# omerbt/Splice

Hardware: AMD Instinct MI355X
Metric: opt_steps_per_sec (higher is better)
Workload: dtype bf16

## Files before the change

### include/splice_hip.h

```cpp
#ifndef SPLICE_HIP_H
#define SPLICE_HIP_H
#include <stddef.h>
#include <stdint.h>

#ifdef __cplusplus
extern "C" {
#endif

typedef uint16_t splice_bf16;
typedef void* splice_stream_t;

#define SPLICE_OK 0
#define SPLICE_ERR_ARG -1
#define SPLICE_ERR_HIP -2
#define SPLICE_ERR_STATE -3
#define SPLICE_ERR_NOMEM -4

int splice_version(void);
int splice_dev_switches(void);
const char* splice_last_error(void);

typedef struct splice_gemm_epilogue {
    const float* bias;
    const float* resid;
// ... 281 lines not shown
                       float* out_f32, size_t os, splice_bf16* out_bf, splice_bf16* pre_bf, const splice_bf16* aux, size_t ps, int pre_lo,
                       splice_stream_t stream);

typedef struct splice_gen_conv_args {
    const float* in;
    const float* w;
    const float* bias;
    float* out;
    size_t in_nstride, in_cstride, out_nstride, out_cstride, w_jstride, w_cstride, p_nstride;
    int N, Cin, Hi, Wi, Cout, Ho, Wo, ks, stride, pad;
    int reflect, act, transposed, accumulate;
    float* ws;
    size_t ws_floats;
    int p_group, defer_reduce;
} splice_gen_conv_args;
#define SPLICE_GEN_CONV_FORM_INTS 5
int splice_gen_conv(const splice_gen_conv_args* args, int* form_out, splice_stream_t stream);
int splice_gen_conv_pair(const splice_gen_conv_args* a, const splice_gen_conv_args* b, int* forms_out, splice_stream_t stream);
int splice_gen_conv_reflect_dgrad(const splice_gen_conv_args* args, float* pad_scratch, size_t scratch_floats, splice_stream_t stream);

typedef struct splice_gen_wgrad_args {
    const float* x;
    const float* dy;
    float* ws;
    size_t ws_floats;
    size_t x_nstride, x_cstride, dy_nstride, dy_cstride;
    int N, Cin, Hi, Wi, Cout, Ho, Wo, ks, stride, pad, reflect;
} splice_gen_wgrad_args;
#define SPLICE_GEN_WGRAD_FORM_INTS 6
size_t splice_gen_conv_wgrad_ws_floats(int N, int Cin, int Cout, int ks, int Ho, int Wo);
int splice_gen_conv_wgrad(const splice_gen_wgrad_args* args, float* dw, int accumulate, int n_img, size_t p_nstride, int* form_out,
                          splice_stream_t stream);
int splice_gen_wgrad_reduce(const float* partials, int n, int chunks, float* dw, int accumulate, int n_img, size_t p_nstride, splice_stream_t stream);

typedef struct splice_gen_bn_args {
    float* y;
    float* out;
    size_t y_nstride, out_nstride;
    int N, C, HW, batch;
    const float* gamma;
    const float* beta;
    float eps, slope;
    size_t p_nstride;
    float* part;
    size_t part_floats;
    float* mean;
    float* rstd;
    const float* up_src;
    float* up_d_src;
    size_t up_src_ns, up_d_src_ns;
    int up_c0, up_h, up_w, up_Ho, up_Wo;
    const float* slabs;
    const float* bias;
    int ksplit;
    const float* da;
    float* dy;
    size_t da_nstride, dy_nstride;
    float* dgamma;
    float* dbeta;
    int accumulate;
    const float* da_slabs;
    int da_ksplit, da_accumulate;
    float* pre_y;
    size_t pre_y_ns;
    const float* pre_slabs;
    const float* pre_bias;
// ... 30 lines not shown
```

### splice_amd/_lib.py

```python
import ctypes as C
import os

_HERE = os.path.dirname(os.path.abspath(__file__))
LIB_PATH = os.path.join(_HERE, "libsplice_hip.so")

_lib = None


class GemmEpilogue(C.Structure):
    _fields_ = [
        ("bias", C.c_void_p), ("resid", C.c_void_p), ("ldr", C.c_int), ("resid_mod", C.c_int),
        ("out_f32", C.c_void_p), ("ldo", C.c_int),
        ("out_bf", C.c_void_p), ("ldbf", C.c_int),
        ("out_bf_t", C.c_void_p), ("ldt", C.c_int),
        ("out_pre", C.c_void_p), ("ldp", C.c_int), ("pre_row_lo", C.c_int),
        ("aux", C.c_void_p), ("ldaux", C.c_int),
        ("out_f32_cols", C.c_void_p), ("ld_cols", C.c_int), ("col_lo", C.c_int), ("col_hi", C.c_int),
        ("alpha", C.c_float), ("ksplit", C.c_int), ("slab_stride", C.c_longlong),
        ("rd_other", C.c_void_p), ("ld_rd", C.c_int), ("rd_rows", C.c_int), ("rowdot", C.c_void_p),
        ("row_scale", C.c_void_p), ("col_scale", C.c_void_p),
        ("out_f8", C.c_void_p), ("ld8", C.c_int),
        ("out_f8_t", C.c_void_p), ("ldt8", C.c_int),
    ]

# ... 79 lines not shown
    "splice_gemm_nt_fp8": ([_u, _vp, _i, _vp, _i, _i, _i, _i, C.POINTER(GemmEpilogue), _vp], _i),
    "splice_quantize_rows_fp8": ([_vp, _i, _vp, _i, _vp, _i, _i, _vp], _i),
    "splice_gemm_splitk_slabs": ([_i, _i], _i),
    "splice_gemm_force_tile": ([_i], _i),
    "splice_attention_variant": ([_i], _i),
    "splice_attention_qfold": ([_i], _i),
    "splice_attention_bwd_variant": ([_i], _i),
    "splice_layernorm_fwd": ([_vp, _vp, _vp, _vp, _vp, _vp, _i, _i, _f, _vp], _i),
    "splice_layernorm_bwd": ([_vp, _vp, _vp, _vp, _vp, _vp, _vp, _vp, _i, _i, _vp], _i),
    "splice_attention_fwd": ([_vp, _vp, _i, _i, _i, _i, _i, _i, _f, _vp, _vp, _vp], _i),
    "splice_attention_fwd_fp8": ([_vp, _vp, _i, _i, _i, _i, _i, _i, _f, _vp, _vp, _vp], _i),
    "splice_attention_bwd": ([_vp, _vp, _i, _i, _i, _i, _i, _i, _f, _vp, _vp, _vp, _vp, _vp, _vp, _vp], _i),
    "splice_attention_probs": ([_vp, _i, _i, _i, _i, _i, _f, _vp, _vp, _vp], _i),
    "splice_augment_structure": ([_vp, _vp, _vp, _i, _i, _i, _i, C.POINTER(C.c_int), C.POINTER(C.c_float), _f, _vp], _i),
    "splice_keys_selfsim_ws_bytes": ([_i, _i], _sz),
    "splice_keys_selfsim_fwd": ([_vp, _i, _i, _i, _f, _vp, _vp, _vp], _i),
    "splice_keys_selfsim_bwd": ([_vp, _vp, _i, _i, _f, _vp, _i, _i, _vp, _vp], _i),
    "splice_mse": ([_vp, _i, _vp, _i, _i, _i, _f, _vp, _vp, _i, _vp], _i),
    "splice_selfsim_loss_pairs_ws_bytes": ([_i, _i, _i], _sz),
    "splice_selfsim_loss_pairs": ([_vp, _vp, _i, _sz, _vp, _i, _sz, _i, _i, _i, _f, _vp, _i, _f, _vp, _sz, _vp, _i, _sz, _vp, _vp], _i),
    "splice_mse_pairs": ([_vp, _i, _sz, _vp, _i, _sz, _i, _i, _f, _f, _vp, _sz, _vp, _i, _sz, _i, _vp, _vp], _i),
    "splice_total_loss_pairs": ([_vp, _sz, _i, _f, _f, _f, _f, _f, _vp, _i, _i, _i, _i, _i, _vp, _i, _i, _vp], _i),
    "splice_attn_cls_fwd": ([_vp, _vp, _i, _i, _i, _i, _i, _i, _f, _vp, _vp, _vp], _i),
    "splice_attn_cls_bwd": ([_vp, _vp, _i, _i, _i, _i, _i, _i, _f, _vp, _vp, _i, _sz, _vp, _vp], _i),
    "splice_ln_rows_fwd": ([_vp, _sz, _vp, _vp, _vp, _sz, _vp, _vp, _sz, _i, _i, _f, _vp, _i, _sz, _vp, _vp, _sz, _vp], _i),
    "splice_ln_rows_bwd": ([_vp, _sz, _vp, _sz, _vp, _vp, _vp, _sz, _vp, _vp, _i, _i, _i, _sz, _vp], _i),
    "splice_rows_finish": ([_i, _vp, _i, _sz, _i, _i, _vp, _vp, _sz, _vp, _sz, _vp, _vp, _vp, _sz, _i, _vp], _i),
    "splice_gen_conv": ([C.POINTER(GenConvArgs), C.POINTER(_i), _vp], _i),
    "splice_gen_conv_pair": ([C.POINTER(GenConvArgs), C.POINTER(GenConvArgs), C.POINTER(_i), _vp], _i),
    "splice_gen_conv_reflect_dgrad": ([C.POINTER(GenConvArgs), _vp, _sz, _vp], _i),
    "splice_gen_conv_wgrad_ws_floats": ([_i, _i, _i, _i, _i, _i], _sz),
    "splice_gen_conv_wgrad": ([C.POINTER(GenWgradArgs), _vp, _i, _i, _sz, C.POINTER(_i), _vp], _i),
    "splice_gen_wgrad_reduce": ([_vp, _i, _i, _vp, _i, _i, _sz, _vp], _i),
    "splice_gen_bn_small_instance": ([_i], _i),
    "splice_gen_bn_form": ([_i, _i, _sz, _i, C.POINTER(_i)], _i),
    "splice_gen_bn_part_floats": ([_i, _i], _sz),
    "splice_gen_bn_fwd": ([C.POINTER(GenBnArgs), _vp], _i),
    "splice_gen_bn_bwd": ([C.POINTER(GenBnArgs), _vp], _i),
    "splice_gen_upsample2x_fwd": ([_vp, _sz, _vp, _sz, _i, _i, _i, _i, _i, _i, _vp], _i),
    "splice_gen_upsample2x_bwd": ([_vp, _sz, _vp, _sz, _i, _i, _i, _i, _i, _i, _vp], _i),
    "splice_gen_sigmoid_bias_part_floats": ([_i, _i], _sz),
    "splice_gen_sigmoid_bwd_bias": ([_vp, _vp, _vp, _i, _i, _i, _vp, _sz, _sz, _i, C.POINTER(_i), _vp], _i),
    "splice_patchify": ([_vp, _vp, _i, _i, _i, _i, _i, _i, _vp], _i),
    "splice_unpatchify": ([_vp, _vp, _i, _i, _i, _i, _i, _i, _vp], _i),
    "splice_cast_f32_bf16": ([_vp, _vp, _sz, _vp], _i),
    "splice_cast_bf16_f32": ([_vp, _vp, _sz, _vp], _i),
    "splice_transpose_f32_bf16": ([_vp, _vp, _i, _i, _i, _vp], _i),
    "splice_resize_bilinear_fwd": ([_vp, _vp, _i, _i, _i, _i, _i, _vp], _i),
    "splice_resize_bilinear_bwd": ([_vp, _vp, _i, _i, _i, _i, _i, _vp], _i),
    "splice_vit_create": ([_i, _i, _i, _i, C.POINTER(_vp)], _i),
    "splice_vit_destroy": ([_vp], None),
    "splice_vit_set_param": ([_vp, C.c_char_p, _vp, C.c_longlong, _vp], _i),
    "splice_vit_params_complete": ([_vp], _i),
    "splice_vit_enable_fp8": ([_vp, _vp], _i),
    "splice_vit_ctx_create": ([_vp, _i, _i, _i, _vp, _i, _vp, C.POINTER(_vp)], _i),
    "splice_vit_ctx_destroy": ([_vp], None),
    "splice_vit_ctx_info": ([_vp, C.POINTER(_i), C.POINTER(_i), C.POINTER(_i)], _i),
    "splice_vit_ctx_set_top_cls_only": ([_vp, _i], _i),
    "splice_vit_ctx_set_fp8": ([_vp, _i], _i),
    "splice_vit_forward": ([_vp, _vp, _i, _vp], _i),
    "splice_vit_forward_ex": ([_vp, _vp, _i, _i, _vp], _i),
    "splice_vit_forward_passes": ([_vp, _vp, _i, _i, _i, _i, _vp], _i),
    "splice_vit_get_tensor": ([_vp, _i, _i, C.POINTER(_vp)], _i),
    "splice_vit_qscale": ([_vp], C.c_float),
    "splice_vit_read_tensor": ([_vp, _i, _i, _vp, _sz, _vp], _i),
    "splice_vit_backward": ([_vp, _i, _i, C.POINTER(_vp), C.POINTER(_vp), C.POINTER(_vp), _vp, _i, _vp], _i),
# ... 102 lines not shown
```

### splice_amd/csrc/capi.hip

```cpp
#include <stdarg.h>
#include <stdio.h>

#include "gen_kernels.h"
#include "kernels.h"

static thread_local char g_err[512] = "";

void splice_set_error(const char* fmt, ...) {
    va_list ap;
    va_start(ap, fmt);
    vsnprintf(g_err, sizeof(g_err), fmt, ap);
    va_end(ap);
}

static int finish(int rc, const char* what) {
    if (rc != SPLICE_OK) {
        splice_set_error("%s: invalid argument", what);
        return rc;
    }
    const hipError_t e = hipGetLastError();
    if (e != hipSuccess) {
        splice_set_error("%s: HIP error %d (%s)", what, (int)e, hipGetErrorString(e));
        return SPLICE_ERR_HIP;
    }
// ... 248 lines not shown
}
size_t splice_gen_conv_wgrad_ws_floats(int N, int Cin, int Cout, int ks, int Ho, int Wo) {
    if (N < 1 || Cin < 1 || Cout < 1 || ks < 1 || Ho < 1 || Wo < 1) return 0;
    int ppc = 0, cpi = 0;
    return (size_t)wgrad_chunks(N, Ho, Wo, &ppc, &cpi) * Cout * Cin * ks * ks;
}
int splice_gen_conv_wgrad(const splice_gen_wgrad_args* args, float* dw, int accumulate, int n_img, size_t p_nstride, int* form_out, splice_stream_t stream) {
    const char* who = "splice_gen_conv_wgrad";
    if (!gen_wgrad_args_ok(args) || !dw || !args->ws) return finish(SPLICE_ERR_ARG, who);
    const size_t n = (size_t)args->Cout * args->Cin * args->ks * args->ks;
    if (n > 0x7fffffffULL || args->ws_floats < splice_gen_conv_wgrad_ws_floats(args->N, args->Cin, args->Cout, args->ks, args->Ho, args->Wo))
        return finish(SPLICE_ERR_ARG, who);
    if (p_nstride ? (n_img != args->N || p_nstride < n) : n_img != 1) return finish(SPLICE_ERR_ARG, who);
    WgradArgs a = {};
    a.x = args->x; a.dy = args->dy; a.ws = args->ws;
    a.x_nstride = args->x_nstride; a.x_cstride = args->x_cstride; a.dy_nstride = args->dy_nstride; a.dy_cstride = args->dy_cstride;
    a.N = args->N; a.Cin = args->Cin; a.Hi = args->Hi; a.Wi = args->Wi; a.Cout = args->Cout; a.Ho = args->Ho; a.Wo = args->Wo;
    a.ks = args->ks; a.stride = args->stride; a.pad = args->pad; a.reflect = args->reflect;
    WgradBatchPair pair = {};
    int chunks = 0;
    int rc = conv_wgrad_add(&pair, a, &chunks);
    if (rc != SPLICE_OK) return finish(rc, who);
    WgradReduceAll r = {};
    r.count = 1; r.n[0] = (int)n; r.chunks[0] = chunks; r.ws_off[0] = 0; r.dw_off[0] = 0;
    if (form_out) {
        const WgradBatch& b = pair.tile.count ? pair.tile : pair.big.count ? pair.big : pair.small;
        form_out[0] = pair.tile.count ? 2 : pair.big.count ? 1 : 0;
        form_out[1] = b.d[0].variant;
        form_out[2] = b.d[0].pix_per_chunk;
        form_out[3] = chunks;
        form_out[4] = !((reinterpret_cast<size_t>(args->ws) | reinterpret_cast<size_t>(dw)) & 15) && p_nstride % 4 == 0 && n % 4 == 0;
        form_out[5] = b.total_wgs;
    }
    rc = conv_wgrad_batched_launch(pair, ST(stream));
    if (rc != SPLICE_OK) return finish(rc, who);
    return finish(wgrad_reduce_all_launch(r, args->ws, dw, accumulate, ST(stream), n_img, p_nstride), who);
}

int splice_gen_wgrad_reduce(const float* partials, int n, int chunks, float* dw, int accumulate, int n_img, size_t p_nstride, splice_stream_t stream) {
    const char* who = "splice_gen_wgrad_reduce";
    if (!partials || !dw || n < 1 || chunks < 0 || n_img < 1 || n_img > 65535 || (long long)n * (chunks > 0 ? chunks : 1) > 0x7fffffffLL) return finish(SPLICE_ERR_ARG, who);
    if (p_nstride ? (chunks % n_img || p_nstride < (size_t)n) : n_img != 1) return finish(SPLICE_ERR_ARG, who);
    WgradReduceAll r = {};
    r.count = 1; r.n[0] = n; r.chunks[0] = chunks; r.ws_off[0] = 0; r.dw_off[0] = 0;
    return finish(wgrad_reduce_all_launch(r, partials, dw, accumulate, ST(stream), n_img, p_nstride), who);
}

int splice_gen_bn_small_instance(int mask) { return finish(bn_small_force_instance(mask), "splice_gen_bn_small_instance"); }
int splice_gen_bn_form(int HW, int N, size_t p_nstride, int batch, int* out) {
    if (HW < 1 || N < 1 || batch < 0 || !out) return finish(SPLICE_ERR_ARG, "splice_gen_bn_form");
    const BnForm f = bn_form(HW, N, p_nstride, batch);
    out[0] = (int)f.kind; out[1] = f.hosts_pre; out[2] = f.fwd_takes_slabs; out[3] = f.bwd_takes_slabs;
    out[4] = f.fwd_fuses_upsample; out[5] = f.bwd_fuses_upsample; out[6] = f.sign_from_y;
    return SPLICE_OK;
}
size_t splice_gen_bn_part_floats(int N, int C) { return N < 1 || C < 1 ? 0 : (size_t)bn_part_floats(N, C); }
static bool gen_bn_fill(const splice_gen_bn_args* g, bool bwd, BnArgs* a, BnUpsample* up, BnPre* pre, BnSlabs* sl) {
    if (!g || !g->y || !g->out || !g->gamma || !g->mean || !g->rstd) return false;
    if (g->N < 1 || g->C < 1 || g->HW < 1 || g->N > 65535 || g->C > 65535 || g->batch < 0 || g->batch > 8) return false;
    if (g->batch && (g->N % g->batch || (g->N != g->batch && !g->p_nstride))) return false;
    if (g->N > 1 && (g->y_nstride < (size_t)g->C * g->HW || g->out_nstride < (size_t)g->C * g->HW)) return false;
    const BnForm f = bn_form(g->HW, g->N, g->p_nstride, g->batch);
    const bool two_stage = f.kind == BnForm::TWO_STAGE || f.kind == BnForm::TWO_STAGE_VEC;
    if (two_stage && (!g->part || g->part_floats < (size_t)bn_part_floats(g->N, g->C))) return false;
    if (!bwd && !g->beta) return false;
    if (bwd && ((f.sign_from_y && !g->beta) || !g->da || !g->dy || !g->dgamma || !g->dbeta)) return false;
    if (bwd && g->N > 1 && (g->da_nstride < (size_t)g->C * g->HW || g->dy_nstride < (size_t)g->C * g->HW)) return false;
    a->y = g->y; a->y_nstride = g->y_nstride; a->out = g->out; a->out_nstride = g->out_nstride;
    a->N = g->N; a->C = g->C; a->HW = g->HW; a->gamma = g->gamma; a->beta = g->beta; a->eps = g->eps; a->slope = g->slope;
    a->p_nstride = g->p_nstride; a->batch = g->batch; a->part = g->part; a->mean = g->mean; a->rstd = g->rstd;
// ... 95 lines not shown
```

### splice_amd/csrc/gen_kernels.h

```cpp
#pragma once
#include "common.h"

struct ConvArgs {
    const float* in;
    const float* w;
    const float* bias;
    float* out;
    size_t in_nstride, in_cstride, out_nstride, out_cstride;
    size_t w_jstride, w_cstride;
    size_t p_nstride;
    int N, Cin, Hi, Wi, Cout, Ho, Wo;
    int ks, stride, pad;
    int reflect;
    int act;
    int transposed;
    int accumulate;
    float* ws;
    size_t ws_floats;
    int ksplit;
    int p_group;
    int defer_reduce;
};
int conv_launch(const ConvArgs& a, hipStream_t s, int* ksplit_out = nullptr);
void conv_form_report(const ConvArgs& a, int* form);
int conv_pair_launch(ConvArgs a, ConvArgs b, hipStream_t s, int* ksplit_a = nullptr, int* ksplit_b = nullptr);
int conv_reflect_dgrad_launch(ConvArgs a, float* pad_scratch, hipStream_t s);

struct WgradArgs {
    const float* x;
    const float* dy;
    float* ws;
    size_t x_nstride, x_cstride, dy_nstride, dy_cstride;
    int N, Cin, Hi, Wi, Cout, Ho, Wo, ks, stride, pad;
    int pix_per_chunk, chunks_per_img;
    int reflect;
};
int wgrad_chunks(int N, int Ho, int Wo, int* pix_per_chunk, int* chunks_per_img);
constexpr int WGRAD_BATCH_MAX = 32;
struct WgradDesc {
    const float* x; const float* dy; float* ws;
    uint32_t x_nstride, x_cstride, dy_nstride, dy_cstride;
    uint16_t Cin, Cout, Hi, Wi, Ho, Wo;
    uint8_t ks, stride, pad, variant;
    uint16_t pix_per_chunk, chunks_per_img;
    uint32_t wg_begin, chunks;
    uint32_t reflect;
};
struct WgradBatch { int count; int total_wgs; WgradDesc d[WGRAD_BATCH_MAX]; };
struct WgradBatchPair { WgradBatch small, big, tile; };
int conv_wgrad_add(WgradBatchPair* b, WgradArgs a, int* chunks_out);
int conv_wgrad_batched_launch(const WgradBatchPair& b, hipStream_t s);

constexpr int WGRAD_MAX_LAYERS = 64;
struct WgradReduceAll {
    long long prefix[WGRAD_MAX_LAYERS + 1];
    long long ws_off[WGRAD_MAX_LAYERS];
    long long dw_off[WGRAD_MAX_LAYERS];
    int n[WGRAD_MAX_LAYERS], chunks[WGRAD_MAX_LAYERS];
    long long total;
    int count;
    unsigned char vec[WGRAD_MAX_LAYERS];
};
int wgrad_reduce_all_launch(const WgradReduceAll& d, const float* ws, float* grads, int accumulate, hipStream_t s, int n_img = 1, size_t p_nstride = 0);

int bn_part_floats(int N, int C);
struct BnUpsample {
    const float* src = nullptr; size_t src_ns = 0;
    float* d_src = nullptr; size_t d_src_ns = 0;
    int c0 = 0, h = 0, w = 0, Ho = 0, Wo = 0;
};
struct BnPre {
    const float* y = nullptr; size_t y_ns = 0;
    const float* slabs = nullptr; int ksplit = 0;
    const float* bias = nullptr;
    const float* gamma = nullptr; const float* beta = nullptr;
    float* mean = nullptr; float* rstd = nullptr;
    float slope = 0.2f;
    int C = 0;
    float* dy = nullptr;
    float* dgamma = nullptr; float* dbeta = nullptr;
};
struct BnSlabs {
    const float* slabs = nullptr;
    int ksplit = 0, accumulate = 0;
// ... 53 lines not shown
```

### splice_amd/csrc/gen_wgrad.hip

```cpp
#include "gen_device.h"
#include <cstdlib>

constexpr int WG_PC = 64;
constexpr int WG_LD = WG_PC + 2;
constexpr int WG_XS_FLOATS = 3 * 16 * WG_LD;
constexpr int WG_DS_FLOATS = 8 * 16 * WG_LD;
template <int KS, int NI, bool ROWS = false>
__device__ __forceinline__ void conv_wgrad_body(const WgradArgs& a, int chunk, int ktile_in, float* Xs, float* Ds) {
    constexpr int T = ROWS ? KS : KS * KS;
    constexpr int CK = (ROWS || KS == 3) ? 4 : 16;
    constexpr int KT = CK * T;
    const int ktile = ROWS ? ktile_in / KS : ktile_in;
    const int krow = ROWS ? ktile_in % KS : 0;
    constexpr int NJ = (KT + 15) / 16;
    constexpr int PC = WG_PC;
    constexpr int LD = WG_LD;
    constexpr int NQ = (NI * NJ + 3) / 4;
    constexpr int NA = KT / 4;
    constexpr int ND = NI * 16 * PC / 256;
    const int tid = threadIdx.x, lane = tid & 63, wave = tid >> 6;
    const int c0 = ktile * CK;
    const int HWo = a.Ho * a.Wo;
    const int chunks_per_img = a.chunks_per_img;
    const int img = chunk / chunks_per_img, ch_in_img = chunk % chunks_per_img;
    const float* x = a.x + (size_t)img * a.x_nstride + (size_t)c0 * a.x_cstride;
    const float* dy = a.dy + (size_t)img * a.dy_nstride;
    f32x4 acc[NQ];
#pragma unroll
    for (int q = 0; q < NQ; ++q) acc[q] = f32x4{0.f, 0.f, 0.f, 0.f};
    for (int e = tid; e < (NJ * 16 - KT) * LD; e += 256) Xs[KT * LD + e] = 0.f;
    const int pl = tid & 63;
    const int p_begin = ch_in_img * a.pix_per_chunk;
    const int p_end = min(p_begin + a.pix_per_chunk, HWo);
    const int wave_g = (KS == 3 && NI == 8) ? __builtin_amdgcn_readfirstlane(wave) : wave;
    int g_coff[NA], g_dy[NA], g_dx[NA];
    unsigned g_cok = 0;
#pragma unroll
    for (int i = 0; i < NA; ++i) {
        const int k = wave_g + 4 * i;
        const int cl = k / T, tap = k % T;
        g_coff[i] = (int)(cl * a.x_cstride);
        g_dy[i] = (ROWS ? krow : tap / KS) - a.pad;
        g_dx[i] = (ROWS ? tap : tap % KS) - a.pad;
        if (c0 + cl < a.Cin) g_cok |= 1u << i;
    }
    float xv[NA], dv[ND];
    const __amdgpu_buffer_rsrc_t rx = __builtin_amdgcn_make_buffer_rsrc(const_cast<float*>(x), 0, 0x7FFFFFFF, 0x00020000);
    const __amdgpu_buffer_rsrc_t rdy = __builtin_amdgcn_make_buffer_rsrc(const_cast<float*>(dy), 0, 0x7FFFFFFF, 0x00020000);
    int d_vo[ND];
#pragma unroll
    for (int t = 0; t < ND; ++t) {
        const int e = tid + 256 * t;
        const int n = e / PC, q = e % PC;
        d_vo[t] = n < a.Cout ? (int)((n * a.dy_cstride + q) * 4) : (int)0x80000000;
    }
    auto fetch = [&](int pb) {
        const int p = pb + pl;
        const bool pvalid = p < p_end;
        const int oy = pvalid ? p / a.Wo : 0, ox = pvalid ? p % a.Wo : 0;
        const int by = oy * a.stride, bx = ox * a.stride;
#pragma unroll
        for (int i = 0; i < NA; ++i) {
            int sy = by + g_dy[i], sx = bx + g_dx[i];
            if (a.reflect) {
                sy = sy < 0 ? -sy : (sy >= a.Hi ? 2 * (a.Hi - 1) - sy : sy);
                sx = sx < 0 ? -sx : (sx >= a.Wi ? 2 * (a.Wi - 1) - sx : sx);
            }
            const bool ok = pvalid && ((g_cok >> i) & 1u) && (unsigned)sy < (unsigned)a.Hi && (unsigned)sx < (unsigned)a.Wi;
            const int vo = ok ? (g_coff[i] + sy * a.Wi + sx) * 4 : (int)0x80000000;
            xv[i] = __builtin_bit_cast(float, __builtin_amdgcn_raw_buffer_load_b32(rx, vo, 0, 0));
        }
        if (pb + PC <= p_end) {
            const int so = __builtin_amdgcn_readfirstlane(pb * 4);
#pragma unroll
            for (int t = 0; t < ND; ++t) dv[t] = __builtin_bit_cast(float, __builtin_amdgcn_raw_buffer_load_b32(rdy, d_vo[t], so, 0));
        } else {
#pragma unroll
            for (int t = 0; t < ND; ++t) {
                const int e = tid + 256 * t;
                const int n = e / PC, q = e % PC;
                const int pp = pb + q;
                dv[t] = (n < a.Cout && pp < p_end) ? dy[(size_t)n * a.dy_cstride + pp] : 0.f;
            }
        }
    };
    fetch(p_begin);
    constexpr int WB = 4, NB = PC / 4 / WB;
    [[maybe_unused]] int lds_rd = (lane & 15) * LD + (lane >> 4);
    for (int pb = p_begin; pb < p_end; pb += PC) {
        if constexpr (NI < 4) asm volatile("" : "+v"(lds_rd));
        __syncthreads();
#pragma unroll
        for (int i = 0; i < NA; ++i) Xs[(wave + 4 * i) * LD + pl] = xv[i];
#pragma unroll
        for (int t = 0; t < ND; ++t) {
            const int e = tid + 256 * t;
            Ds[(e / PC) * LD + (e % PC)] = dv[t];
        }
        __syncthreads();
        if (pb + PC < p_end) fetch(pb + PC);
#pragma unroll
        for (int q = 0; q < NQ; ++q) {
            const int pair = wave + 4 * q;
            if (pair < NI * NJ) {
                const int fi = pair / NJ, fj = pair % NJ;
                if constexpr (NI >= 4) {
#pragma unroll
                    for (int s4 = 0; s4 < PC / 4; ++s4) {
                        const float av = Ds[(fi * 16 + (lane & 15)) * LD + s4 * 4 + (lane >> 4)];
                        const float bv = Xs[(fj * 16 + (lane & 15)) * LD + s4 * 4 + (lane >> 4)];
                        acc[q] = mfma4(av, bv, acc[q]);
                    }
                } else {
                    const int d_rd = lds_rd + fi * 16 * LD, x_rd = lds_rd + fj * 16 * LD;
                    float af[2][WB], bf[2][WB];
#pragma unroll
                    for (int t = 0; t < WB; ++t) { af[0][t] = Ds[d_rd + t * 4]; bf[0][t] = Xs[x_rd + t * 4]; }
#pragma unroll
                    for (int b = 0; b < NB; ++b) {
                        if (b + 1 < NB) {
#pragma unroll
                            for (int t = 0; t < WB; ++t) { af[(b + 1) & 1][t] = Ds[d_rd + ((b + 1) * WB + t) * 4]; bf[(b + 1) & 1][t] = Xs[x_rd + ((b + 1) * WB + t) * 4]; }
                        }
                        __builtin_amdgcn_sched_barrier(0);
#pragma unroll
                        for (int t = 0; t < WB; ++t) acc[q] = mfma4(af[b & 1][t], bf[b & 1][t], acc[q]);
                        __builtin_amdgcn_sched_barrier(0);
                    }
                }
            }
        }
    }
    constexpr int TT = KS * KS;
    float* ws = a.ws + (size_t)chunk * a.Cout * a.Cin * TT;
#pragma unroll
    for (int q = 0; q < NQ; ++q) {
        const int pair = wave + 4 * q;
        if (pair < NI * NJ) {
            const int fi = pair / NJ, fj = pair % NJ;
            const int k = fj * 16 + (lane & 15);
            const int cl = k / T, tap = k % T;
            if (k < KT && c0 + cl < a.Cin) {
#pragma unroll
                for (int r = 0; r < 4; ++r) {
                    const int n = fi * 16 + (lane >> 4) * 4 + r;
                    if (n < a.Cout) ws[((size_t)n * a.Cin + c0 + cl) * TT + (ROWS ? krow * KS + tap : tap)] = acc[q][r];
                }
            }
        }
    }
}

__device__ __forceinline__ void wgrad_loaded(float& x) { asm volatile("" : "+v"(x) : : "memory"); }
template <class Load>
__device__ __forceinline__ float wgrad_chunk_sum(int chunks, Load&& ld) {
    float s0 = 0.f, s1 = 0.f, s2 = 0.f, s3 = 0.f;
    int c = 0;
#pragma unroll 1
    for (; c + 31 < chunks; c += 32) {
        float v[32];
#pragma unroll
        for (int u = 0; u < 32; ++u) v[u] = ld(c + u);
#pragma unroll
        for (int u = 0; u < 32; ++u) wgrad_loaded(v[u]);
#pragma unroll
        for (int u = 0; u < 32; u += 4) { s0 += v[u]; s1 += v[u + 1]; s2 += v[u + 2]; s3 += v[u + 3]; }
    }
    for (; c + 15 < chunks; c += 16) {
        float v[16];
#pragma unroll
// ... 71 lines not shown
            const float4 v0 = *reinterpret_cast<const float4*>(p + (size_t)c * n), v1 = *reinterpret_cast<const float4*>(p + (size_t)(c + 1) * n),
                         v2 = *reinterpret_cast<const float4*>(p + (size_t)(c + 2) * n), v3 = *reinterpret_cast<const float4*>(p + (size_t)(c + 3) * n);
            a0.x += v0.x; a0.y += v0.y; a0.z += v0.z; a0.w += v0.w;
            a1.x += v1.x; a1.y += v1.y; a1.z += v1.z; a1.w += v1.w;
            a2.x += v2.x; a2.y += v2.y; a2.z += v2.z; a2.w += v2.w;
            a3.x += v3.x; a3.y += v3.y; a3.z += v3.z; a3.w += v3.w;
        }
        for (; c < chunks; ++c) {
            const float4 v0 = *reinterpret_cast<const float4*>(p + (size_t)c * n);
            a0.x += v0.x; a0.y += v0.y; a0.z += v0.z; a0.w += v0.w;
        }
        s.x = (a0.x + a1.x) + (a2.x + a3.x); s.y = (a0.y + a1.y) + (a2.y + a3.y);
        s.z = (a0.z + a1.z) + (a2.z + a3.z); s.w = (a0.w + a1.w) + (a2.w + a3.w);
        float4* q4 = reinterpret_cast<float4*>(q);
        if (accumulate) { const float4 o = *q4; s.x = o.x + s.x; s.y = o.y + s.y; s.z = o.z + s.z; s.w = o.w + s.w; }
        *q4 = s;
        return;
    }
    const float s = wgrad_chunk_sum(chunks, [&](int c) { return p[(size_t)c * n]; });
    *q = accumulate ? *q + s : s;
}

int wgrad_chunks(int N, int Ho, int Wo, int* pix_per_chunk, int* chunks_per_img) {
    const int HWo = Ho * Wo;
    int ppc = 512;
    if (HWo <= 1024) ppc = 256;
    if (HWo <= 256) ppc = 64;
    if (HWo > 128 * 512) ppc = (cdiv(HWo, 128) + 63) / 64 * 64;
    *pix_per_chunk = ppc;
    *chunks_per_img = cdiv(HWo, ppc);
    return N * *chunks_per_img;
}

template <bool BIG>
__global__ __launch_bounds__(256, 2) void conv_wgrad_batched_kernel(WgradBatch b) {
    __shared__ float Xs[WG_XS_FLOATS];
    __shared__ float Ds[(BIG ? 8 : 2) * 16 * WG_LD];
    int l = 0;
#pragma unroll 1
    while (l + 1 < b.count && blockIdx.x >= b.d[l + 1].wg_begin) ++l;
    const WgradDesc& d = b.d[l];
    WgradArgs a;
    a.x = d.x; a.dy = d.dy; a.ws = d.ws;
    a.x_nstride = d.x_nstride; a.x_cstride = d.x_cstride; a.dy_nstride = d.dy_nstride; a.dy_cstride = d.dy_cstride;
    a.N = 0; a.Cin = d.Cin; a.Hi = d.Hi; a.Wi = d.Wi; a.Cout = d.Cout; a.Ho = d.Ho; a.Wo = d.Wo;
    a.ks = d.ks; a.stride = d.stride; a.pad = d.pad; a.pix_per_chunk = d.pix_per_chunk; a.chunks_per_img = d.chunks_per_img;
    a.reflect = (int)d.reflect;
    const int local = blockIdx.x - d.wg_begin;
    const int chunk = local % d.chunks, ktile = local / d.chunks;
    if (BIG) {
        switch (d.variant) {
            case 2: conv_wgrad_body<1, 4>(a, chunk, ktile, Xs, Ds); break;
            case 3: conv_wgrad_body<1, 8>(a, chunk, ktile, Xs, Ds); break;
            case 6: conv_wgrad_body<3, 4>(a, chunk, ktile, Xs, Ds); break;
            case 7: conv_wgrad_body<3, 8>(a, chunk, ktile, Xs, Ds); break;
            case 10: conv_wgrad_body<5, 4, true>(a, chunk, ktile, Xs, Ds); break;
            case 11: conv_wgrad_body<5, 8, true>(a, chunk, ktile, Xs, Ds); break;
            case 14: conv_wgrad_body<7, 4, true>(a, chunk, ktile, Xs, Ds); break;
            default: conv_wgrad_body<7, 8, true>(a, chunk, ktile, Xs, Ds); break;
        }
    } else {
        switch (d.variant) {
            case 0: conv_wgrad_body<1, 1>(a, chunk, ktile, Xs, Ds); break;
            case 1: conv_wgrad_body<1, 2>(a, chunk, ktile, Xs, Ds); break;
            case 4: conv_wgrad_body<3, 1>(a, chunk, ktile, Xs, Ds); break;
            case 5: conv_wgrad_body<3, 2>(a, chunk, ktile, Xs, Ds); break;
            case 8: conv_wgrad_body<5, 1, true>(a, chunk, ktile, Xs, Ds); break;
            case 9: conv_wgrad_body<5, 2, true>(a, chunk, ktile, Xs, Ds); break;
            case 12: conv_wgrad_body<7, 1, true>(a, chunk, ktile, Xs, Ds); break;
            default: conv_wgrad_body<7, 2, true>(a, chunk, ktile, Xs, Ds); break;
        }
    }
}

constexpr int WT_CK = 8, WT_NJ = 5, WT_PH = 6, WT_PLANE = WT_PH * CT_PW, WT_PE = WT_CK * WT_PLANE, WT_NP = (WT_PE + 255) / 256;
template <int NI>
__device__ __forceinline__ void conv_wgrad_tile_body(const WgradDesc& d, int chunk, int ktile, int nb , float* Ps) {
    const int tid = threadIdx.x, lane = tid & 63, wave = __builtin_amdgcn_readfirstlane(tid >> 6);
    const int Cin = d.Cin, Cout = d.Cout, Hi = d.Hi, Wi = d.Wi, Ho = d.Ho, Wo = d.Wo, pad = d.pad;
    const int img = chunk / d.chunks_per_img, strip = chunk % d.chunks_per_img;
    const int tiles_x = (Wo + CT_TW - 1) / CT_TW, tiles_y = (Ho + 3) / 4, T = tiles_x * tiles_y;
    const int t_begin = (int)((long long)strip * T / d.chunks_per_img), t_end = (int)((long long)(strip + 1) * T / d.chunks_per_img);
    const int c0 = ktile * WT_CK;
    const float* x = d.x + (size_t)img * d.x_nstride + (size_t)c0 * d.x_cstride;
    const float* dy = d.dy + (size_t)img * d.dy_nstride;
    const __amdgpu_buffer_rsrc_t rx = __builtin_amdgcn_make_buffer_rsrc(const_cast<float*>(x), 0, 0x7FFFFFFF, 0x00020000);
    const __amdgpu_buffer_rsrc_t rdy = __builtin_amdgcn_make_buffer_rsrc(const_cast<float*>(dy), 0, 0x7FFFFFFF, 0x00020000);
    int p_rel[WT_NP];
#pragma unroll
    for (int j = 0; j < WT_NP; ++j) {
        const int e = tid + 256 * j;
        const int c = e / WT_PLANE, rem = e % WT_PLANE, r = rem / CT_PW, xx = rem % CT_PW;
        p_rel[j] = (e < WT_PE && c0 + c < Cin) ? (int)(c * d.x_cstride + (unsigned)(r * Wi + xx)) * 4 : (int)0x80000000;
    }
    int b_base[WT_NJ];
#pragma unroll
    for (int jf = 0; jf < WT_NJ; ++jf) {
        const int j = jf * 16 + (lane & 15);
        const int cl = j / 9, tap = j % 9;
        b_base[jf] = (j < WT_CK * 9 ? cl * WT_PLANE + (tap / 3) * CT_PW + tap % 3 : 0) + wave * CT_PW + 4 * (lane >> 4);
    }
    int dy_off[NI];
#pragma unroll
    for (int fi = 0; fi < NI; ++fi) {
        const int n = nb + fi * 16 + (lane & 15);
        dy_off[fi] = n < Cout ? (int)(n * d.dy_cstride) * 4 : (int)0x80000000;
// ... 115 lines not shown
    else conv_wgrad_tile_body<2>(d, chunk, ktile, nb, Ps);
}
static bool wgrad_tile_ok(const WgradArgs& a) {
    static const int on = getenv("SPLICE_WGRAD_TILE") ? atoi(getenv("SPLICE_WGRAD_TILE")) : 1;
    constexpr int min_px = 40000;
    return on && a.ks == 3 && a.stride == 1 && a.Wo >= 64 && (long long)a.Ho * a.Wo > min_px && a.Hi == a.Ho && a.Wi == a.Wo && a.pad == 1 &&
           (size_t)a.Cin * a.x_cstride <= 0x1fffffffULL && (size_t)a.Cout * a.dy_cstride <= 0x1fffffffULL;
}

int conv_wgrad_add(WgradBatchPair* pair, WgradArgs a, int* chunks_out) {
    const bool tile = wgrad_tile_ok(a);
    WgradBatch* b = tile ? &pair->tile : a.Cout > 32 ? &pair->big : &pair->small;
    if (a.Cout > 128 || (a.ks != 1 && a.ks != 3 && a.ks != 5 && a.ks != 7) || b->count >= WGRAD_BATCH_MAX) return SPLICE_ERR_ARG;
    if ((size_t)a.Cin * a.x_cstride > 0x7fffffffULL || a.x_nstride > 0xffffffffULL || a.dy_nstride > 0xffffffffULL) return SPLICE_ERR_ARG;
    if (a.Hi > 65535 || a.Wi > 65535 || a.Cin > 65535) return SPLICE_ERR_ARG;
    const int chunks = wgrad_chunks(a.N, a.Ho, a.Wo, &a.pix_per_chunk, &a.chunks_per_img);
    const int CK = tile ? WT_CK : a.ks == 1 ? 16 : 4;
    const int ktiles = cdiv(a.Cin, CK) * (a.ks >= 5 ? a.ks : 1) * (tile ? cdiv(a.Cout, 32) : 1);
    const int ni = cdiv(a.Cout, 16);
    WgradDesc& d = b->d[b->count++];
    d.x = a.x; d.dy = a.dy; d.ws = a.ws;
    d.x_nstride = (uint32_t)a.x_nstride; d.x_cstride = (uint32_t)a.x_cstride; d.dy_nstride = (uint32_t)a.dy_nstride; d.dy_cstride = (uint32_t)a.dy_cstride;
    d.Cin = (uint16_t)a.Cin; d.Cout = (uint16_t)a.Cout; d.Hi = (uint16_t)a.Hi; d.Wi = (uint16_t)a.Wi; d.Ho = (uint16_t)a.Ho; d.Wo = (uint16_t)a.Wo;
    d.ks = (uint8_t)a.ks; d.stride = (uint8_t)a.stride; d.pad = (uint8_t)a.pad;
    d.variant = (uint8_t)((a.ks == 3 ? 4 : a.ks == 5 ? 8 : a.ks == 7 ? 12 : 0) + (ni <= 1 ? 0 : ni <= 2 ? 1 : ni <= 4 ? 2 : 3));
    if (tile) d.variant = (uint8_t)(ni < 2 ? 1 : 2);
    d.reflect = (uint32_t)(a.reflect ? 1 : 0);
    d.pix_per_chunk = (uint16_t)a.pix_per_chunk; d.chunks_per_img = (uint16_t)a.chunks_per_img;
    d.wg_begin = (uint32_t)b->total_wgs; d.chunks = (uint32_t)chunks;
    b->total_wgs += chunks * ktiles;
    if (chunks_out) *chunks_out = chunks;
    return SPLICE_OK;
}
int conv_wgrad_batched_launch(const WgradBatchPair& p, hipStream_t s) {
    if (p.big.count > 0) SPLICE_LAUNCH(conv_wgrad_batched_kernel<true>, dim3((unsigned)p.big.total_wgs), dim3(256), 0, s, p.big);
    if (p.small.count > 0) SPLICE_LAUNCH(conv_wgrad_batched_kernel<false>, dim3((unsigned)p.small.total_wgs), dim3(256), 0, s, p.small);
    if (p.tile.count > 0) SPLICE_LAUNCH(conv_wgrad_tile_kernel, dim3((unsigned)p.tile.total_wgs), dim3(256), 0, s, p.tile);
    return SPLICE_OK;
}

int wgrad_reduce_all_launch(const WgradReduceAll& d0, const float* ws, float* grads, int accumulate, hipStream_t s, int n_img, size_t p_nstride) {
    if (d0.count < 1 || d0.count > WGRAD_MAX_LAYERS) return SPLICE_ERR_ARG;
    WgradReduceAll d = d0;
    static const int vec_on = getenv("SPLICE_WGRAD_REDUCE_VEC") ? atoi(getenv("SPLICE_WGRAD_REDUCE_VEC")) : 1;
    const bool base_ok = vec_on && !((reinterpret_cast<size_t>(ws) | reinterpret_cast<size_t>(grads)) & 15) && p_nstride % 4 == 0;
    d.prefix[0] = 0;
    for (int i = 0; i < d.count; ++i) {
        const bool v = base_ok && d.n[i] % 4 == 0 && d.ws_off[i] % 4 == 0 && d.dw_off[i] % 4 == 0;
        d.vec[i] = v ? 1 : 0;
        d.prefix[i + 1] = d.prefix[i] + (v ? d.n[i] / 4 : d.n[i]);
    }
    d.total = d.prefix[d.count];
    SPLICE_LAUNCH(wgrad_reduce_all_kernel, dim3((unsigned)((d.total + 255) / 256), p_nstride ? n_img : 1), dim3(256), 0, s, d, ws, grads, accumulate,
                       n_img, p_nstride);
    return SPLICE_OK;
}
```

Baseline: 270.6.

## Give each wave its own output rows in big wgrad kernel with register-blocked MFMA

Result: no change. 271.6, median of 6 (+0.4%).

```diff
diff --git a/include/splice_hip.h b/include/splice_hip.h
--- a/include/splice_hip.h
+++ b/include/splice_hip.h
@@ -337,6 +337,7 @@
 int splice_gen_conv_wgrad(const splice_gen_wgrad_args* args, float* dw, int accumulate, int n_img, size_t p_nstride, int* form_out,
                           splice_stream_t stream);
 int splice_gen_wgrad_reduce(const float* partials, int n, int chunks, float* dw, int accumulate, int n_img, size_t p_nstride, splice_stream_t stream);
+int splice_gen_wgrad_big_reference(int on);
 
 typedef struct splice_gen_bn_args {
     float* y;
diff --git a/splice_amd/_lib.py b/splice_amd/_lib.py
--- a/splice_amd/_lib.py
+++ b/splice_amd/_lib.py
@@ -135,6 +135,7 @@
     "splice_gen_conv_wgrad_ws_floats": ([_i, _i, _i, _i, _i, _i], _sz),
     "splice_gen_conv_wgrad": ([C.POINTER(GenWgradArgs), _vp, _i, _i, _sz, C.POINTER(_i), _vp], _i),
     "splice_gen_wgrad_reduce": ([_vp, _i, _i, _vp, _i, _i, _sz, _vp], _i),
+    "splice_gen_wgrad_big_reference": ([_i], _i),
     "splice_gen_bn_small_instance": ([_i], _i),
     "splice_gen_bn_form": ([_i, _i, _sz, _i, C.POINTER(_i)], _i),
     "splice_gen_bn_part_floats": ([_i, _i], _sz),
diff --git a/splice_amd/csrc/capi.hip b/splice_amd/csrc/capi.hip
--- a/splice_amd/csrc/capi.hip
+++ b/splice_amd/csrc/capi.hip
@@ -304,10 +304,11 @@
         form_out[4] = !((reinterpret_cast<size_t>(args->ws) | reinterpret_cast<size_t>(dw)) & 15) && p_nstride % 4 == 0 && n % 4 == 0;
         form_out[5] = b.total_wgs;
     }
-    rc = conv_wgrad_batched_launch(pair, ST(stream));
+    rc = conv_wgrad_batched_launch(pair, ST(stream), wgrad_big_reference_forced());
     if (rc != SPLICE_OK) return finish(rc, who);
     return finish(wgrad_reduce_all_launch(r, args->ws, dw, accumulate, ST(stream), n_img, p_nstride), who);
 }
+int splice_gen_wgrad_big_reference(int on) { return finish(wgrad_big_force_reference(on), "splice_gen_wgrad_big_reference"); }
 
 int splice_gen_wgrad_reduce(const float* partials, int n, int chunks, float* dw, int accumulate, int n_img, size_t p_nstride, splice_stream_t stream) {
     const char* who = "splice_gen_wgrad_reduce";
diff --git a/splice_amd/csrc/gen_kernels.h b/splice_amd/csrc/gen_kernels.h
--- a/splice_amd/csrc/gen_kernels.h
+++ b/splice_amd/csrc/gen_kernels.h
@@ -49,7 +49,9 @@
 struct WgradBatch { int count; int total_wgs; WgradDesc d[WGRAD_BATCH_MAX]; };
 struct WgradBatchPair { WgradBatch small, big, tile; };
 int conv_wgrad_add(WgradBatchPair* b, WgradArgs a, int* chunks_out);
-int conv_wgrad_batched_launch(const WgradBatchPair& b, hipStream_t s);
+int conv_wgrad_batched_launch(const WgradBatchPair& b, hipStream_t s, bool big_reference = false);
+int wgrad_big_force_reference(int on);
+bool wgrad_big_reference_forced();
 
 constexpr int WGRAD_MAX_LAYERS = 64;
 struct WgradReduceAll {
diff --git a/splice_amd/csrc/gen_wgrad.hip b/splice_amd/csrc/gen_wgrad.hip
--- a/splice_amd/csrc/gen_wgrad.hip
+++ b/splice_amd/csrc/gen_wgrad.hip
@@ -1,12 +1,20 @@
 #include "gen_device.h"
+#include <atomic>
 #include <cstdlib>
 
 constexpr int WG_PC = 64;
 constexpr int WG_LD = WG_PC + 2;
 constexpr int WG_XS_FLOATS = 3 * 16 * WG_LD;
 constexpr int WG_DS_FLOATS = 8 * 16 * WG_LD;
-template <int KS, int NI, bool ROWS = false>
+__device__ __forceinline__ const float* wgrad_uniform(const float* p) {
+    const unsigned long long v = reinterpret_cast<unsigned long long>(p);
+    const unsigned lo = (unsigned)__builtin_amdgcn_readfirstlane((int)(unsigned)v), hi = (unsigned)__builtin_amdgcn_readfirstlane((int)(unsigned)(v >> 32));
+    return reinterpret_cast<const float*>(((unsigned long long)hi << 32) | lo);
+}
+template <int KS, int NI, bool ROWS = false, bool REF = false>
 __device__ __forceinline__ void conv_wgrad_body(const WgradArgs& a, int chunk, int ktile_in, float* Xs, float* Ds) {
+    constexpr bool OWN = NI >= 4 && !REF;
+    constexpr int FI = NI / 4;
     constexpr int T = ROWS ? KS : KS * KS;
     constexpr int CK = (ROWS || KS == 3) ? 4 : 16;
     constexpr int KT = CK * T;
@@ -25,6 +33,10 @@
     const int img = chunk / chunks_per_img, ch_in_img = chunk % chunks_per_img;
     const float* x = a.x + (size_t)img * a.x_nstride + (size_t)c0 * a.x_cstride;
     const float* dy = a.dy + (size_t)img * a.dy_nstride;
+    if constexpr (OWN) {
+        x = wgrad_uniform(x);
+        dy = wgrad_uniform(dy);
+    }
     f32x4 acc[NQ];
 #pragma unroll
     for (int q = 0; q < NQ; ++q) acc[q] = f32x4{0.f, 0.f, 0.f, 0.f};
@@ -32,7 +44,7 @@
     const int pl = tid & 63;
     const int p_begin = ch_in_img * a.pix_per_chunk;
     const int p_end = min(p_begin + a.pix_per_chunk, HWo);
-    const int wave_g = (KS == 3 && NI == 8) ? __builtin_amdgcn_readfirstlane(wave) : wave;
+    const int wave_g = (OWN || (KS == 3 && NI == 8)) ? __builtin_amdgcn_readfirstlane(wave) : wave;
     int g_coff[NA], g_dy[NA], g_dx[NA];
     unsigned g_cok = 0;
 #pragma unroll
@@ -47,12 +59,18 @@
     float xv[NA], dv[ND];
     const __amdgpu_buffer_rsrc_t rx = __builtin_amdgcn_make_buffer_rsrc(const_cast<float*>(x), 0, 0x7FFFFFFF, 0x00020000);
     const __amdgpu_buffer_rsrc_t rdy = __builtin_amdgcn_make_buffer_rsrc(const_cast<float*>(dy), 0, 0x7FFFFFFF, 0x00020000);
-    int d_vo[ND];
-#pragma unroll
-    for (int t = 0; t < ND; ++t) {
-        const int e = tid + 256 * t;
-        const int n = e / PC, q = e % PC;
-        d_vo[t] = n < a.Cout ? (int)((n * a.dy_cstride + q) * 4) : (int)0x80000000;
+    [[maybe_unused]] int d_vo[OWN ? 1 : ND];
+    [[maybe_unused]] int d_v0 = 0;
+    [[maybe_unused]] const unsigned d_ts = (unsigned)(16 * a.dy_cstride);
+    if constexpr (OWN) {
+        d_v0 = (int)((wave * a.dy_cstride + pl) * 4);
+    } else {
+#pragma unroll
+        for (int t = 0; t < ND; ++t) {
+            const int e = tid + 256 * t;
+            const int n = e / PC, q = e % PC;
+            d_vo[t] = n < a.Cout ? (int)((n * a.dy_cstride + q) * 4) : (int)0x80000000;
+        }
     }
     auto fetch = [&](int pb) {
         const int p = pb + pl;
@@ -70,7 +88,14 @@
             const int vo = ok ? (g_coff[i] + sy * a.Wi + sx) * 4 : (int)0x80000000;
             xv[i] = __builtin_bit_cast(float, __builtin_amdgcn_raw_buffer_load_b32(rx, vo, 0, 0));
         }
-        if (pb + PC <= p_end) {
+        if constexpr (OWN) {
+            const int so = __builtin_amdgcn_readfirstlane(pb * 4);
+            const int vo_p = pvalid ? d_v0 : (int)0x80000000;
+#pragma unroll
+            for (int t = 0; t < ND; ++t)
+                dv[t] = __builtin_bit_cast(float, __builtin_amdgcn_raw_buffer_load_b32(rdy, wave_g + 4 * t < a.Cout ? vo_p : (int)0x80000000,
+                                                                                         (int)((unsigned)so + (unsigned)t * d_ts), 0));
+        } else if (pb + PC <= p_end) {
             const int so = __builtin_amdgcn_readfirstlane(pb * 4);
 #pragma unroll
             for (int t = 0; t < ND; ++t) dv[t] = __builtin_bit_cast(float, __builtin_amdgcn_raw_buffer_load_b32(rdy, d_vo[t], so, 0));
@@ -85,20 +110,61 @@
         }
     };
     fetch(p_begin);
-    constexpr int WB = 4, NB = PC / 4 / WB;
+    constexpr int WB = (OWN && FI * NJ >= 6) ? 2 : 4, NB = PC / 4 / WB;
     [[maybe_unused]] int lds_rd = (lane & 15) * LD + (lane >> 4);
+    [[maybe_unused]] int lds_rd_d = lds_rd + wave * (FI * 16 * LD);
+    [[maybe_unused]] int lds_wr = wave * LD + pl;
     for (int pb = p_begin; pb < p_end; pb += PC) {
         if constexpr (NI < 4) asm volatile("" : "+v"(lds_rd));
+        if constexpr (OWN) asm volatile("" : "+v"(lds_rd), "+v"(lds_rd_d), "+v"(lds_wr), "+v"(d_v0));
         __syncthreads();
-#pragma unroll
-        for (int i = 0; i < NA; ++i) Xs[(wave + 4 * i) * LD + pl] = xv[i];
-#pragma unroll
-        for (int t = 0; t < ND; ++t) {
-            const int e = tid + 256 * t;
-            Ds[(e / PC) * LD + (e % PC)] = dv[t];
+        if constexpr (OWN) {
+#pragma unroll
+            for (int i = 0; i < NA; ++i) Xs[lds_wr + i * 4 * LD] = xv[i];
+#pragma unroll
+            for (int t = 0; t < ND; ++t) Ds[lds_wr + t * 4 * LD] = dv[t];
+        } else {
+#pragma unroll
+            for (int i = 0; i < NA; ++i) Xs[(wave + 4 * i) * LD + pl] = xv[i];
+#pragma unroll
+            for (int t = 0; t < ND; ++t) {
+                const int e = tid + 256 * t;
+                Ds[(e / PC) * LD + (e % PC)] = dv[t];
+            }
         }
         __syncthreads();
         if (pb + PC < p_end) fetch(pb + PC);
+        if constexpr (OWN) {
+            static_assert(FI * NJ == NQ, "accumulator (i, j) = acc[i * NJ + j]");
+            float af[2][WB][FI], bf[2][WB][NJ];
+#pragma unroll
+            for (int t = 0; t < WB; ++t) {
+#pragma unroll
+                for (int i = 0; i < FI; ++i) af[0][t][i] = Ds[lds_rd_d + i * 16 * LD + t * 4];
+#pragma unroll
+                for (int j = 0; j < NJ; ++j) bf[0][t][j] = Xs[lds_rd + j * 16 * LD + t * 4];
+            }
+#pragma unroll
+            for (int b = 0; b < NB; ++b) {
+                if (b + 1 < NB) {
+#pragma unroll
+                    for (int t = 0; t < WB; ++t) {
+#pragma unroll
+                        for (int i = 0; i < FI; ++i) af[(b + 1) & 1][t][i] = Ds[lds_rd_d + i * 16 * LD + ((b + 1) * WB + t) * 4];
+#pragma unroll
+                        for (int j = 0; j < NJ; ++j) bf[(b + 1) & 1][t][j] = Xs[lds_rd + j * 16 * LD + ((b + 1) * WB + t) * 4];
+                    }
+                }
+                __builtin_amdgcn_sched_barrier(0);
+#pragma unroll
+                for (int t = 0; t < WB; ++t)
+#pragma unroll
+                    for (int i = 0; i < FI; ++i)
+#pragma unroll
+                        for (int j = 0; j < NJ; ++j) acc[i * NJ + j] = mfma4(af[b & 1][t][i], bf[b & 1][t][j], acc[i * NJ + j]);
+                __builtin_amdgcn_sched_barrier(0);
+            }
+        } else {
 #pragma unroll
         for (int q = 0; q < NQ; ++q) {
             const int pair = wave + 4 * q;
@@ -130,12 +196,13 @@
                 }
             }
         }
+        }
     }
     constexpr int TT = KS * KS;
     float* ws = a.ws + (size_t)chunk * a.Cout * a.Cin * TT;
 #pragma unroll
     for (int q = 0; q < NQ; ++q) {
-        const int pair = wave + 4 * q;
+        const int pair = OWN ? wave * NQ + q : wave + 4 * q;
         if (pair < NI * NJ) {
             const int fi = pair / NJ, fj = pair % NJ;
             const int k = fj * 16 + (lane & 15);
@@ -273,8 +340,8 @@
     return N * *chunks_per_img;
 }
 
-template <bool BIG>
-__global__ __launch_bounds__(256, 2) void conv_wgrad_batched_kernel(WgradBatch b) {
+template <bool BIG, bool REF>
+__device__ __forceinline__ void conv_wgrad_batched_run(const WgradBatch& b) {
     __shared__ float Xs[WG_XS_FLOATS];
     __shared__ float Ds[(BIG ? 8 : 2) * 16 * WG_LD];
     int l = 0;
@@ -291,14 +358,14 @@
     const int chunk = local % d.chunks, ktile = local / d.chunks;
     if (BIG) {
         switch (d.variant) {
-            case 2: conv_wgrad_body<1, 4>(a, chunk, ktile, Xs, Ds); break;
-            case 3: conv_wgrad_body<1, 8>(a, chunk, ktile, Xs, Ds); break;
-            case 6: conv_wgrad_body<3, 4>(a, chunk, ktile, Xs, Ds); break;
-            case 7: conv_wgrad_body<3, 8>(a, chunk, ktile, Xs, Ds); break;
-            case 10: conv_wgrad_body<5, 4, true>(a, chunk, ktile, Xs, Ds); break;
-            case 11: conv_wgrad_body<5, 8, true>(a, chunk, ktile, Xs, Ds); break;
-            case 14: conv_wgrad_body<7, 4, true>(a, chunk, ktile, Xs, Ds); break;
-            default: conv_wgrad_body<7, 8, true>(a, chunk, ktile, Xs, Ds); break;
+            case 2: conv_wgrad_body<1, 4, false, REF>(a, chunk, ktile, Xs, Ds); break;
+            case 3: conv_wgrad_body<1, 8, false, REF>(a, chunk, ktile, Xs, Ds); break;
+            case 6: conv_wgrad_body<3, 4, false, REF>(a, chunk, ktile, Xs, Ds); break;
+            case 7: conv_wgrad_body<3, 8, false, REF>(a, chunk, ktile, Xs, Ds); break;
+            case 10: conv_wgrad_body<5, 4, true, REF>(a, chunk, ktile, Xs, Ds); break;
+            case 11: conv_wgrad_body<5, 8, true, REF>(a, chunk, ktile, Xs, Ds); break;
+            case 14: conv_wgrad_body<7, 4, true, REF>(a, chunk, ktile, Xs, Ds); break;
+            default: conv_wgrad_body<7, 8, true, REF>(a, chunk, ktile, Xs, Ds); break;
         }
     } else {
         switch (d.variant) {
@@ -313,6 +380,9 @@
         }
     }
 }
+template <bool BIG>
+__global__ __launch_bounds__(256, BIG ? 3 : 2) void conv_wgrad_batched_kernel(WgradBatch b) { conv_wgrad_batched_run<BIG, false>(b); }
+__global__ __launch_bounds__(256, 2) void conv_wgrad_big_reference_kernel(WgradBatch b) { conv_wgrad_batched_run<true, true>(b); }
 
 constexpr int WT_CK = 8, WT_NJ = 5, WT_PH = 6, WT_PLANE = WT_PH * CT_PW, WT_PE = WT_CK * WT_PLANE, WT_NP = (WT_PE + 255) / 256;
 template <int NI>
@@ -494,8 +564,16 @@
     if (chunks_out) *chunks_out = chunks;
     return SPLICE_OK;
 }
-int conv_wgrad_batched_launch(const WgradBatchPair& p, hipStream_t s) {
-    if (p.big.count > 0) SPLICE_LAUNCH(conv_wgrad_batched_kernel<true>, dim3((unsigned)p.big.total_wgs), dim3(256), 0, s, p.big);
+static std::atomic<int> g_wgrad_big_reference{0};
+int wgrad_big_force_reference(int on) {
+    if (on != 0 && on != 1) return SPLICE_ERR_ARG;
+    g_wgrad_big_reference.store(on);
+    return SPLICE_OK;
+}
+bool wgrad_big_reference_forced() { return g_wgrad_big_reference.load(std::memory_order_relaxed) != 0; }
+int conv_wgrad_batched_launch(const WgradBatchPair& p, hipStream_t s, bool big_reference) {
+    if (p.big.count > 0 && big_reference) SPLICE_LAUNCH(conv_wgrad_big_reference_kernel, dim3((unsigned)p.big.total_wgs), dim3(256), 0, s, p.big);
+    else if (p.big.count > 0) SPLICE_LAUNCH(conv_wgrad_batched_kernel<true>, dim3((unsigned)p.big.total_wgs), dim3(256), 0, s, p.big);
     if (p.small.count > 0) SPLICE_LAUNCH(conv_wgrad_batched_kernel<false>, dim3((unsigned)p.small.total_wgs), dim3(256), 0, s, p.small);
     if (p.tile.count > 0) SPLICE_LAUNCH(conv_wgrad_tile_kernel, dim3((unsigned)p.tile.total_wgs), dim3(256), 0, s, p.tile);
     return SPLICE_OK;
```
